# boqian333/E2ENet-Medical

Hardware: AMD Instinct MI355X
Metric: voxels/sec (train step fwd+bwd+update), 128^3 patch 32ch density=0.2 (higher is better)
Workload: dtype f32 (fp16x2 split products, f32 accumulate); 1 GPU; BraTS-shaped 4-modal 128^3 patches, shiftConvPP base 32, K=4, DSFF density 0.2, batch 2 per GPU, fwd+loss+bwd+clip+SGD+mask step, dense (parity) wgrad; parallelism=dp1

## Files before the change

e2enet_medical_amd/_lib.py:

```python
import ctypes as C
import os

_HERE = os.path.dirname(os.path.abspath(__file__))
LIB_PATH = os.environ.get("E2E_LIB_PATH") or os.path.join(_HERE, "csrc", "libe2e_hip.so")

KNOWN_ENV = frozenset({
    "E2E_CONV_MM", "E2E_MM_GRID", "E2E_MM_GEOM", "E2E_MM_PAIRQ", "E2E_CONV_DENSE", "E2E_CONV_SPARSE2", "E2E_CONV_PERSIST", "E2E_CONV_WGS",
    "E2E_CONV_KSPLIT", "E2E_WG_H2", "E2E_WG_BF3", "E2E_CT_BF3", "E2E_CT_H2",
    "E2E_CONV_DBG", "E2E_MM_STAMPS",
    "E2E_LIB_PATH", "E2E_STRICT_ENV", "E2E_DENSE_MIN_DENSITY", "E2E_MM_MIN_DENSITY", "E2E_WGRAD_STREAM", "E2E_LANES", "E2E_GRAPHS",
    "E2E_GRAPH_MAX_VOXELS", "E2E_PLAN_CACHE_GB", "E2E_SW_BLOCKING", "E2E_FORCE_DIST",
    "E2E_CPU_THREADS", "E2E_BENCH_DRY", "E2E_BENCH_DRY_FAIL_RANK", "E2E_BENCH_ALL_LAUNCHES",
})


def check_env(environ=None, strict=None):
    environ = os.environ if environ is None else environ
    unknown = sorted(k for k in environ if k.startswith("E2E_") and k not in KNOWN_ENV)
    if not unknown:
        return
    msg = ("unknown E2E_* environment variable(s) %s: not read by this build (known: %s)"
           % (", ".join(unknown), ", ".join(sorted(KNOWN_ENV))))
    if strict is None:
        strict = environ.get("E2E_STRICT_ENV") == "1"
    if strict:
        raise RuntimeError(msg)
    import warnings
    warnings.warn(msg + "; set E2E_STRICT_ENV=1 to refuse instead", RuntimeWarning, stacklevel=2)


class InChan(C.Structure):
    _fields_ = [("ptr", C.c_void_p), ("scale", C.c_void_p), ("shift", C.c_void_p),
                ("nstride", C.c_longlong), ("ab_nstride", C.c_int), ("dshift", C.c_int),
                ("slope", C.c_float), ("reserved", C.c_int)]


class OutChan(C.Structure):
    _fields_ = [("ptr", C.c_void_p), ("nstride", C.c_longlong), ("dshift", C.c_int), ("accumulate", C.c_int)]


class InSumChan(C.Structure):
    _fields_ = [("y", C.c_void_p), ("scale", C.c_void_p), ("shift", C.c_void_p), ("mean", C.c_void_p), ("rstd", C.c_void_p),
                ("part", C.c_void_p), ("nstride", C.c_longlong), ("part_nstride", C.c_longlong), ("ab_nstride", C.c_int),
                ("slope", C.c_float)]


class ParamEntry(C.Structure):
    _fields_ = [("param", C.c_void_p), ("grad", C.c_void_p), ("momentum", C.c_void_p), ("mask", C.c_void_p),
                ("numel", C.c_longlong)]


class SparsePackJob(C.Structure):
    _fields_ = [("w", C.c_void_p), ("wpk", C.c_void_p), ("qslot", C.c_void_p), ("pslot", C.c_void_p), ("quads", C.c_void_p),
                ("woff", C.c_void_p), ("groups", C.c_int), ("nchunks", C.c_int), ("wq_stride", C.c_int), ("wp_stride", C.c_int),
                ("reverse", C.c_int), ("kmax", C.c_int)]


class MmPackJob(C.Structure):
    _fields_ = [("w", C.c_void_p), ("quads", C.c_void_p), ("wpk", C.c_void_p), ("w_absmax", C.c_void_p), ("P", C.c_int), ("Q", C.c_int),
                ("wq_stride", C.c_int), ("wp_stride", C.c_int), ("reverse", C.c_int), ("owns_absmax", C.c_int)]


class RangeSrc(C.Structure):
    _fields_ = [("kind", C.c_int), ("C", C.c_int), ("N", C.c_longlong), ("gamma", C.c_void_p), ("beta", C.c_void_p), ("w", C.c_void_p),
                ("wCout", C.c_int), ("wks", C.c_int), ("word", C.c_void_p)]


class RangeJob(C.Structure):
    _fields_ = [("src", RangeSrc * 3), ("out", C.c_void_p)]


assert C.sizeof(MmPackJob) == 56 and C.sizeof(RangeSrc) == 56 and C.sizeof(RangeJob) == 176
assert C.sizeof(InChan) == 48 and C.sizeof(OutChan) == 24 and C.sizeof(ParamEntry) == 40 and C.sizeof(SparsePackJob) == 72 and C.sizeof(InSumChan) == 72

P, I, F, LL = C.c_void_p, C.c_int, C.c_float, C.c_longlong

SIGNATURES = {
    "e2e_last_error": (C.c_char_p, []),
    "e2e_abi_version": (I, []),
    "e2e_last_kernel": (C.c_char_p, []),
    "e2e_conv133_num_partials": (I, [I, I, I, I, I]),
    "e2e_conv133_fwd": (I, [P, I, P, P, P, P, P, I, I, I, I, I, I, I, I, P]),
    "e2e_conv133_fwd_ws_bytes": (LL, [I, I, I, I, I, I, I, I, I]),
    "e2e_conv133_fwd_splitk": (I, [P, I, P, P, P, P, P, I, I, I, I, I, I, I, I, P, LL, P]),
    "e2e_conv133_dgrad": (I, [P, P, P, P, I, I, I, I, I, I, I, I, I, P]),
    "e2e_conv133_dgrad_ws_bytes": (LL, [I, I, I, I, I, I, I, I, I]),
    "e2e_conv133_dgrad_splitk": (I, [P, P, P, P, I, I, I, I, I, I, I, I, I, P, LL, P]),
    "e2e_conv133_dense_ws_bytes": (LL, [I, I, I, I, I, I, I, I, I]),
    "e2e_conv133_sparse_eligible": (I, [I, I, I, I, I, I, I, I]),
    "e2e_conv133_sparse_wpk_floats": (LL, [I, I, I]),
    "e2e_conv133_sparse_plan": (I, [P, I, I, I, P, P, P, P, P, P]),
# ... 150 lines not shown
```

e2enet_medical_amd/csrc/conv133.hip:

```cpp
#include "e2e_common.h"
#include "e2e_split.h"
#include <cstdlib>
#include <cstdio>
#include <type_traits>

#ifdef E2E_CONV_DEBUG
#define CDBG(bit) ((p.dbg & (bit)) != 0)
__device__ unsigned long long g_conv_stamps[1024 * 8];
#define STAMP(var) const unsigned long long var = __builtin_readcyclecounter()
#define STAMP_ADD(i, a, b) st_acc[i] += (b) - (a)
#else
#define STAMP(var)
#define STAMP_ADD(i, a, b)
#define CDBG(bit) false
#endif

namespace {

using namespace e2e;

struct ConvParams {
  const e2e_in_chan_t* chans;
  const float* xin;
  const float* w;
// ... 984 lines not shown
  const bool vec = (DH == 1 && DW == 1) && (p.Wi % 4 == 0);
  switch (kind) {
    case 0:
      if (vec && opw8_knob() == 1 && p.P > 8) return launch_cfg<MODE, 1, 1, 1, 1, 16, 32, 8, 8, 8, 4, 8, 1, 3, 0>(p, st);
      if (vec && opw8_knob() == 2 && p.P > 8) return launch_cfg<MODE, 1, 1, 1, 1, 16, 32, 8, 8, 4, 4, 8, 1, 4, 0>(p, st);
      return vec ? launch_cfg<MODE, 1, 1, 1, 1, 16, 32, 8, 8, 4, 8, 8, 1, 4, 0>(p, st)
                 : launch_cfg<MODE, 1, 1, DH, DW, 16, 32, 8, 8, 4, 8, 8, 0, 4, 0>(p, st);
    case 1:
      return vec ? launch_cfg<MODE, 1, 1, 1, 1, 16, 16, 8, 8, 4, 8, 16, 1>(p, st)
                 : launch_cfg<MODE, 1, 1, DH, DW, 16, 16, 8, 8, 4, 8, 16, 0>(p, st);
    default:
      return vec ? launch_cfg<MODE, 1, 1, 1, 1, 8, 8, 8, 8, 4, 8, 16, 1>(p, st)
                 : launch_cfg<MODE, 1, 1, DH, DW, 8, 8, 8, 8, 4, 8, 16, 0>(p, st);
  }
}

enum TileKind { T32 = 0, T16 = 1, T8 = 2, T16x32S = 3, T8S = 4 };
inline TileKind pick_tile(int Ho, int Wo, int sh, int sw) {
  const bool strided = (sh != 1 || sw != 1);
  const int m = Ho < Wo ? Ho : Wo;
  if (strided) return m > 8 ? T16x32S : T8S;
  if (m > 16) return T32;
  if (m > 8) return T16;
  return T8;
}
inline void tile_dims(TileKind k, int& th, int& tw) {
  switch (k) {
    case T32: th = 16; tw = 32; break;
    case T16: th = 16; tw = 16; break;
    case T8: th = 8; tw = 8; break;
    case T16x32S: th = 16; tw = 32; break;
    default: th = 8; tw = 8; break;
  }
}



int launch_sub(const ConvParams& p, int kind, hipStream_t st) {
  const bool vec = (p.Ws % 4) == 0;
  if (kind == 0)
    return vec ? launch_cfg<2, 1, 1, 1, 1, 16, 32, 8, 8, 4, 8, 8, 1, 4, 0>(p, st)
               : launch_cfg<2, 1, 1, 1, 1, 16, 32, 8, 8, 4, 8, 8, 0, 4, 0>(p, st);
  return vec ? launch_cfg<2, 1, 1, 1, 1, 16, 16, 8, 8, 4, 8, 16, 1>(p, st)
             : launch_cfg<2, 1, 1, 1, 1, 16, 16, 8, 8, 4, 8, 16, 0>(p, st);
}

}

extern "C" int e2e_conv133_num_partials(int Do, int Ho, int Wo, int sh, int sw) {
  int th, tw;
  tile_dims(pick_tile(Ho, Wo, sh, sw), th, tw);
  return Do * e2e::cdiv(Ho, th) * e2e::cdiv(Wo, tw);
}

static int plan_fwd_ksplit(int B, int Cin, int Cout, int Di, int Hi, int Wi, int sd, int sh, int sw) {
  static const int knob = getenv("E2E_CONV_KSPLIT") ? atoi(getenv("E2E_CONV_KSPLIT")) : -1;
  const int Do = (Di - 1) / sd + 1, Ho = (Hi - 1) / sh + 1, Wo = (Wi - 1) / sw + 1;
  const TileKind k = pick_tile(Ho, Wo, sh, sw);
  if (k == T32 || k == T16x32S) return 1;
  int th, tw;
  tile_dims(k, th, tw);
  const int chunks = e2e::cdiv(Cin, 16);
  const long long base = (long long)B * Do * e2e::cdiv(Ho, th) * e2e::cdiv(Wo, tw) * e2e::cdiv(Cout, 32);
  if (knob == 0 || knob == 1) return 1;
  long long ks = knob > 1 ? knob : 1024 / (base > 0 ? base : 1);
  if (ks > 8) ks = 8;
  if (ks > chunks / 2) ks = chunks / 2;
  return ks < 2 ? 1 : (int)ks;
}

extern "C" long long e2e_conv133_fwd_ws_bytes(int B, int Cin, int Cout, int Di, int Hi, int Wi, int sd, int sh, int sw) {
  const int ks = plan_fwd_ksplit(B, Cin, Cout, Di, Hi, Wi, sd, sh, sw);
  if (ks <= 1) return 0;
  const long long Do = (Di - 1) / sd + 1, Ho = (Hi - 1) / sh + 1, Wo = (Wi - 1) / sw + 1;
  return (long long)ks * B * Cout * Do * Ho * Wo * 4;
}

static int conv133_fwd_impl(const e2e_in_chan_t* chans, int Cin, const float* w, const float* bias, const unsigned* live, float* y,
                            double* part, int B, int Cout, int Di, int Hi, int Wi, int sd, int sh, int sw, float* ws,
                            long long ws_bytes, void* stream) {
  E2E_REQUIRE(chans && w && y, "conv133_fwd: null pointer");
  E2E_REQUIRE(B > 0 && Cin > 0 && Cout > 0 && Di > 0 && Hi > 0 && Wi > 0, "conv133_fwd: bad dims");
  E2E_REQUIRE((sd == 1 || sd == 2) && (sh == 1 || sh == 2) && (sw == 1 || sw == 2), "conv133_fwd: stride must be 1 or 2");
  ConvParams p{};
  p.chans = chans; p.xin = nullptr; p.w = w; p.bias = bias; p.live = live; p.y = y; p.part = part; p.outs = nullptr;
  p.P = Cin; p.Q = Cout; p.wq_stride = Cin * 9; p.wp_stride = 9; p.live_words = e2e::cdiv(Cin, 32);
  p.B = B; p.Di = Di; p.Hi = Hi; p.Wi = Wi; p.sd = sd;
  p.Do = (Di - 1) / sd + 1; p.Ho = (Hi - 1) / sh + 1; p.Wo = (Wi - 1) / sw + 1;
  p.Ds = Di; p.Hs = Hi; p.Ws = Wi;
  p.ksplit = 1; p.kpart = nullptr;
  if (ws != nullptr) {
    const long long need = e2e_conv133_fwd_ws_bytes(B, Cin, Cout, Di, Hi, Wi, sd, sh, sw);
    if (need > 0) {
      E2E_REQUIRE(ws_bytes >= need, "conv133_fwd: workspace too small (%lld < %lld bytes)", ws_bytes, need);
      p.ksplit = plan_fwd_ksplit(B, Cin, Cout, Di, Hi, Wi, sd, sh, sw);
      p.kpart = ws;
    }
  }
  hipStream_t st = (hipStream_t)stream;
  const TileKind k = pick_tile(p.Ho, p.Wo, sh, sw);
  if (sh == 1 && sw == 1) return launch_s1<0, 1, 1>(p, k == T32 ? 0 : (k == T16 ? 1 : 2), st);
  if (sh == 2 && sw == 2) {
    if (k == T16x32S && (Wi % 4) == 0) return launch_cfg<0, 2, 2, 1, 1, 16, 32, 4, 16, 4, 8, 8, 1>(p, st);
    if (k == T16x32S) return launch_cfg<0, 2, 2, 1, 1, 16, 32, 4, 16, 4, 8, 8, 0>(p, st);
    return launch_cfg<0, 2, 2, 1, 1, 8, 8, 8, 8, 4, 8, 16, 0>(p, st);
  }
  if (sh == 1 && sw == 2) {
    if (k == T16x32S) return launch_cfg<0, 1, 2, 1, 1, 16, 32, 4, 16, 4, 8, 8, 0>(p, st);
    return launch_cfg<0, 1, 2, 1, 1, 8, 8, 8, 8, 4, 8, 16, 0>(p, st);
  }
  if (k == T16x32S) return launch_cfg<0, 2, 1, 1, 1, 16, 32, 4, 16, 4, 8, 8, 0>(p, st);
  return launch_cfg<0, 2, 1, 1, 1, 8, 8, 8, 8, 4, 8, 16, 0>(p, st);
}

extern "C" int e2e_conv133_fwd(const e2e_in_chan_t* chans, int Cin, const float* w, const float* bias,
                               const unsigned* live, float* y, double* part, int B, int Cout, int Di, int Hi, int Wi,
                               int sd, int sh, int sw, void* stream) {
  return conv133_fwd_impl(chans, Cin, w, bias, live, y, part, B, Cout, Di, Hi, Wi, sd, sh, sw, nullptr, 0, stream);
}

extern "C" int e2e_conv133_fwd_splitk(const e2e_in_chan_t* chans, int Cin, const float* w, const float* bias,
                                      const unsigned* live, float* y, double* part, int B, int Cout, int Di, int Hi, int Wi,
                                      int sd, int sh, int sw, float* ws, long long ws_bytes, void* stream) {
  return conv133_fwd_impl(chans, Cin, w, bias, live, y, part, B, Cout, Di, Hi, Wi, sd, sh, sw, ws, ws_bytes, stream);
}

static int plan_dgrad_ksplit(int B, int Cin, int Cout, int Di, int Hi, int Wi, int sd, int sh, int sw) {
  static const int knob = getenv("E2E_CONV_KSPLIT") ? atoi(getenv("E2E_CONV_KSPLIT")) : -1;
  if (knob == 0 || knob == 1) return 1;
  const bool tiled = (sh == 1 && sw == 1) || (sh == 2 && sw == 2);
  if (!tiled) return 1;
  const TileKind k = pick_tile(Hi, Wi, 1, 1);
  if (k == T32) return 1;
  int th, tw;
  tile_dims(k, th, tw);
  const int chunks = e2e::cdiv(Cout, 16);
  const long long base = (long long)B * Di * e2e::cdiv(Hi, th) * e2e::cdiv(Wi, tw) * e2e::cdiv(Cin, 32);
  long long ks = knob > 1 ? knob : 1024 / (base > 0 ? base : 1);
  if (ks > 8) ks = 8;
  if (ks > chunks / 2) ks = chunks / 2;
  return ks < 2 ? 1 : (int)ks;
}

extern "C" long long e2e_conv133_dgrad_ws_bytes(int B, int Cin, int Cout, int Di, int Hi, int Wi, int sd, int sh, int sw) {
  const int ks = plan_dgrad_ksplit(B, Cin, Cout, Di, Hi, Wi, sd, sh, sw);
  return ks <= 1 ? 0 : (long long)ks * B * Cin * Di * Hi * Wi * 4;
}

static int conv133_dgrad_impl(const float* dy, const float* w, const unsigned* live_t, const e2e_out_chan_t* outs,
                              int B, int Cin, int Cout, int Di, int Hi, int Wi, int sd, int sh, int sw, float* ws,
                              long long ws_bytes, void* stream) {
  E2E_REQUIRE(dy && w && outs, "conv133_dgrad: null pointer");
  E2E_REQUIRE(B > 0 && Cin > 0 && Cout > 0 && Di > 0 && Hi > 0 && Wi > 0, "conv133_dgrad: bad dims");
  E2E_REQUIRE((sd == 1 || sd == 2) && (sh == 1 || sh == 2) && (sw == 1 || sw == 2), "conv133_dgrad: stride must be 1 or 2");
  hipStream_t st = (hipStream_t)stream;
  const int Do = (Di - 1) / sd + 1, Ho = (Hi - 1) / sh + 1, Wo = (Wi - 1) / sw + 1;
  const bool tiled = (sh == 1 && sw == 1) || (sh == 2 && sw == 2);
  if (!tiled) {
    const long long per = (long long)Di * Hi * Wi;
    dim3 grid((unsigned)e2e::cdivll(per, 256), Cin, B);
    e2e::note_kernel("conv133_dgrad_strided_gather");
    hipLaunchKernelGGL(conv133_dgrad_strided_kernel, grid, dim3(256), 0, st, dy, w, outs, B, Cin, Cout, Di, Hi, Wi, Do,
                       Ho, Wo, sd, sh, sw);
    return e2e::check_launch("conv133_dgrad_strided_kernel");
  }
  ConvParams p{};
  p.chans = nullptr; p.xin = dy; p.w = w; p.bias = nullptr; p.live = live_t; p.y = nullptr; p.part = nullptr; p.outs = outs;
  p.P = Cout; p.Q = Cin; p.wq_stride = 9; p.wp_stride = Cin * 9; p.live_words = e2e::cdiv(Cout, 32);
  p.B = B; p.Di = Di; p.Hi = Hi; p.Wi = Wi; p.sd = sd; p.Do = Di; p.Ho = Hi; p.Wo = Wi;
  p.Ds = Do; p.Hs = Ho; p.Ws = Wo;
  p.ksplit = 1; p.kpart = nullptr;
  if (ws != nullptr) {
    const long long need = e2e_conv133_dgrad_ws_bytes(B, Cin, Cout, Di, Hi, Wi, sd, sh, sw);
    if (need > 0) {
      E2E_REQUIRE(ws_bytes >= need, "conv133_dgrad: workspace too small (%lld < %lld bytes)", ws_bytes, need);
      p.ksplit = plan_dgrad_ksplit(B, Cin, Cout, Di, Hi, Wi, sd, sh, sw);
      p.kpart = ws;
    }
  }
  const TileKind k = pick_tile(Hi, Wi, 1, 1);
  const int kind = k == T32 ? 0 : (k == T16 ? 1 : 2);
  if (sh == 1) return launch_s1<1, 1, 1>(p, kind, st);
  if (kind <= 1 && (Hi % 2) == 0 && (Wi % 2) == 0) {
    p.wq_stride = 9; p.wp_stride = Cin * 9;
    return launch_sub(p, kind, st);
  }
  return launch_s1<1, 2, 2>(p, kind, st);
}

extern "C" int e2e_conv133_dgrad(const float* dy, const float* w, const unsigned* live_t, const e2e_out_chan_t* outs,
                                 int B, int Cin, int Cout, int Di, int Hi, int Wi, int sd, int sh, int sw,
                                 void* stream) {
  return conv133_dgrad_impl(dy, w, live_t, outs, B, Cin, Cout, Di, Hi, Wi, sd, sh, sw, nullptr, 0, stream);
}

extern "C" int e2e_conv133_dgrad_splitk(const float* dy, const float* w, const unsigned* live_t, const e2e_out_chan_t* outs,
                                        int B, int Cin, int Cout, int Di, int Hi, int Wi, int sd, int sh, int sw, float* ws,
                                        long long ws_bytes, void* stream) {
  return conv133_dgrad_impl(dy, w, live_t, outs, B, Cin, Cout, Di, Hi, Wi, sd, sh, sw, ws, ws_bytes, stream);
}
```

e2enet_medical_amd/csrc/e2e_common.h:

```cpp
#pragma once
#include <hip/hip_runtime.h>
#include <cstdio>
#include <cstdarg>
#include "e2e_hip.h"

typedef const float __attribute__((address_space(1)))* gfloat_p;

namespace e2e {

void set_error(const char* fmt, ...);
void note_kernel(const char* fmt, ...);

void mm_clock_read(unsigned long long out[2], bool reset);
void wgrad_clock_read(unsigned long long out[2], bool reset);

inline int check_launch(const char* what) {
  hipError_t e = hipGetLastError();
  if (e != hipSuccess) {
    set_error("%s: %s", what, hipGetErrorString(e));
    return E2E_ERR_LAUNCH;
  }
  return E2E_OK;
}

// ... 7 lines not shown

__host__ __device__ inline int cdiv(int a, int b) { return (a + b - 1) / b; }
__host__ __device__ inline long long cdivll(long long a, long long b) { return (a + b - 1) / b; }

__device__ __forceinline__ float in_act(float v, float a, float b, float slope) {
  float u = fmaf(v, a, b);
  return u > 0.f ? u : u * slope;
}

__device__ __forceinline__ float wave_sum_dpp(float v) {
  v += __builtin_bit_cast(float, __builtin_amdgcn_update_dpp(0, __builtin_bit_cast(int, v), 0xB1, 0xF, 0xF, true));
  v += __builtin_bit_cast(float, __builtin_amdgcn_update_dpp(0, __builtin_bit_cast(int, v), 0x4E, 0xF, 0xF, true));
  v += __builtin_bit_cast(float, __builtin_amdgcn_update_dpp(0, __builtin_bit_cast(int, v), 0x141, 0xF, 0xF, true));
  v += __builtin_bit_cast(float, __builtin_amdgcn_update_dpp(0, __builtin_bit_cast(int, v), 0x140, 0xF, 0xF, true));
  v += __shfl_xor(v, 16, 64);
  v += __shfl_xor(v, 32, 64);
  return v;
}

__device__ __forceinline__ double dpp_move_d(double v, const int ctrl_sel) {
  const long long b = __builtin_bit_cast(long long, v);
  int lo = (int)b, hi = (int)(b >> 32);
  switch (ctrl_sel) {
    case 0: lo = __builtin_amdgcn_update_dpp(0, lo, 0xB1, 0xF, 0xF, true); hi = __builtin_amdgcn_update_dpp(0, hi, 0xB1, 0xF, 0xF, true); break;
    case 1: lo = __builtin_amdgcn_update_dpp(0, lo, 0x4E, 0xF, 0xF, true); hi = __builtin_amdgcn_update_dpp(0, hi, 0x4E, 0xF, 0xF, true); break;
    case 2: lo = __builtin_amdgcn_update_dpp(0, lo, 0x141, 0xF, 0xF, true); hi = __builtin_amdgcn_update_dpp(0, hi, 0x141, 0xF, 0xF, true); break;
    default: lo = __builtin_amdgcn_update_dpp(0, lo, 0x140, 0xF, 0xF, true); hi = __builtin_amdgcn_update_dpp(0, hi, 0x140, 0xF, 0xF, true); break;
  }
  return __builtin_bit_cast(double, ((long long)hi << 32) | (unsigned)lo);
}
__device__ __forceinline__ double wave_sum_dpp_d(double v) {
  v += dpp_move_d(v, 0);
  v += dpp_move_d(v, 1);
  v += dpp_move_d(v, 2);
  v += dpp_move_d(v, 3);
  v += __shfl_xor(v, 16, 64);
  v += __shfl_xor(v, 32, 64);
  return v;
}

__device__ __forceinline__ float wave_sum(float v) {
#pragma unroll
  for (int off = 32; off > 0; off >>= 1) v += __shfl_xor(v, off, 64);
  return v;
}
__device__ __forceinline__ double wave_sum_d(double v) {
#pragma unroll
  for (int off = 32; off > 0; off >>= 1) v += __shfl_xor(v, off, 64);
  return v;
}

__device__ __forceinline__ int xcd_remap(int id, int padded_total) {
  int per = padded_total >> 3;
  return (id & 7) * per + (id >> 3);
}

__global__ inline void zero_words_kernel(unsigned* p, long long n) {
  for (long long i = (long long)blockIdx.x * blockDim.x + threadIdx.x; i < n; i += (long long)gridDim.x * blockDim.x) p[i] = 0u;
}
inline void zero_async(void* p, size_t bytes, hipStream_t st) {
  const long long n = (long long)(bytes / 4);
  long long blocks = (n + 255) / 256;
  if (blocks > 2048) blocks = 2048;
  if (blocks < 1) blocks = 1;
  hipLaunchKernelGGL(zero_words_kernel, dim3((unsigned)blocks), dim3(256), 0, st, (unsigned*)p, n);
}

struct WgBf3Params {
  const e2e_in_chan_t* chans;
  const float* dy;
  float* slab;
  int B, Cin, Cout, Di, Hi, Wi, Do, sd;
  int tiles_x, tiles_y, tiles_per_n, tiles_per_chunk;
  int segs;
  int cblocks;
  int geom;
  int h2;
  const unsigned* dy_absmax;
  const unsigned* x_absmax;
};
int launch_wgrad_bf3(const WgBf3Params& p, int nchunks, int pairs, hipStream_t st);
int reduce_slabs(const float* slab, float* dw, long long numel, int nslabs, hipStream_t st);

inline int split_tiles(long long total, int pairs, int target_wgs, int min_tiles, int* tiles_per_chunk) {
  long long want = target_wgs / (pairs > 0 ? pairs : 1);
  if (want < 1) want = 1;
  long long tpc = cdivll(total, want);
  if (tpc < min_tiles) tpc = min_tiles;
  if (tpc > total) tpc = total;
  *tiles_per_chunk = (int)tpc;
  return (int)cdivll(total, tpc);
}
inline int split_tiles_per_item(int tiles_per_n, int B, int pairs, int target_wgs, int min_tiles, int* tiles_per_chunk, int* segs) {
  long long want = target_wgs / (pairs > 0 ? pairs : 1);
  if (want < B) want = B;
  int tpc = cdiv(tiles_per_n, (int)(want / B));
  if (tpc < min_tiles) tpc = min_tiles;
  if (tpc > tiles_per_n) tpc = tiles_per_n;
  *tiles_per_chunk = tpc;
  *segs = cdiv(tiles_per_n, tpc);
  return *segs * B;
}

}
```

e2enet_medical_amd/engine.py:

```python
import contextlib
import ctypes as C
import math
import os
from typing import Dict, List, Optional, Sequence, Tuple

import torch

import numpy as np

from ._lib import lib, InChan, OutChan, ParamEntry, SparsePackJob, InSumChan, MmPackJob, RangeSrc, RangeJob

LRELU_SLOPE = 0.01
IN_EPS = 1e-5
DENSE_MIN_DENSITY = float(os.environ.get("E2E_DENSE_MIN_DENSITY", "0.5"))
WGRAD_STREAM = os.environ.get("E2E_WGRAD_STREAM", "1") != "0"
WGRAD_STREAM_MAX_ELEMS = 40000000
WGRAD_LATE = True
LANES = os.environ.get("E2E_LANES", "1") != "0"
LANE_DIVS = None


def _lane_divs(voxels):
    if LANE_DIVS is not None:
        return LANE_DIVS
# ... 655 lines not shown
        self._region_words_dev = {}
        self._mm_tables = {}
        self._mm_packed = {}
        self._range_table = None
        self._range_key = None
        self.weights_epoch = 0

    def _build_unetpp(self, cfg):
        P = cfg.num_pool
        nodes = {}
        cur = self.input
        for st in range(P + 1):
            stride = (1, 1, 1) if st == 0 else cfg.pool_kernels[st - 1]
            for bi, prefix in enumerate(cfg.encoder_prefixes(st)):
                op = self._add_conv(prefix, [cur], cfg.feats[st], stride if bi == 0 else (1, 1, 1))
                cur = op.out
            nodes[(st, 0)] = cur
            if st == 0:
                continue
            z = P - st
            for m, lvl in cfg.nest_nodes(z):
                j = st - lvl
                up = UpOp(self, "up%d.%d.weight" % (z, m), nodes[(lvl + 1, j - 1)], cfg.feats[lvl], cfg.pool_kernels[lvl])
                self.ops.append(up)
                self.up_ops[up.w_name] = up
                srcs = [nodes[(lvl, j - 1)], up.out]
                if lvl > 0:
                    pool = PoolOp(self, "down%d.%d" % (z, m), nodes[(lvl - 1, j - 1)], cfg.pool_kernels[lvl - 1])
                    self.ops.append(pool)
                    srcs.append(pool.out)
                t = None
                for prefix in cfg.loc_prefixes(z, m):
                    op = self._add_conv(prefix, srcs if t is None else [t], cfg.feats[lvl], (1, 1, 1))
                    t = op.out
                nodes[(lvl, j)] = t
        self.nodes = nodes
        for h in range(4):
            head = HeadOp(self, "seg_outputs.%d.weight" % h, nodes[(h, P - h)], cfg.num_classes)
            self.heads.append(head)
            self.ops.append(head)

    def _build_unet(self, cfg):
        P = cfg.num_pool
        skips, cur = [], self.input
        for st in range(P + 1):
            stride = (1, 1, 1) if st == 0 else cfg.pool_kernels[st - 1]
            for bi, prefix in enumerate(cfg.encoder_prefixes(st)):
                op = self._add_conv(prefix, [cur], cfg.feats[st], stride if bi == 0 else (1, 1, 1))
                cur = op.out
            if st < P:
                skips.append(cur)
        self.nodes = {(st, 0): a for st, a in enumerate(skips)}
        by_u = []
        for u in range(P):
            lvl = P - 1 - u
            up = UpOp(self, "tu.%d.weight" % u, cur, cfg.feats[lvl], cfg.pool_kernels[lvl])
            self.ops.append(up)
            self.up_ops[up.w_name] = up
            t = None
            for prefix in cfg.unet_loc_prefixes(u):
                op = self._add_conv(prefix, [up.out, skips[lvl]] if t is None else [t], cfg.feats[lvl], (1, 1, 1))
                t = op.out
            cur = t
            self.nodes[(lvl, 1)] = t
            head = HeadOp(self, "seg_outputs.%d.weight" % u, t, cfg.num_classes)
            self.ops.append(head)
            by_u.append(head)
        self.heads = [by_u[-1]] + by_u[:-1][::-1]

    def _add_conv(self, prefix, sources, cout, stride):
        op = ConvOp(self, prefix, sources, cout, stride)
        self.ops.append(op)
        self.conv_ops[op.w_name] = op
        return op

    def set_kernel_masks(self, kmasks: Dict[str, torch.Tensor]):
        L = lib()
        self.maps_generation += 1
        self._graphs.clear()
        self._graph_seen.clear()
        self._sparse_jobs = None
        for name, op in list(self.conv_ops.items()) + list(self.up_ops.items()):
            km = kmasks.get(name)
            if isinstance(op, ConvOp):
                op.build_sparse_plans(km)
            if km is None:
                op.live = op.live_t = None
                op.density = 1.0
                continue
            r, cc = km.shape
            op.density = float(km.float().mean().item())
            km = km.to(device=self.device, dtype=torch.uint8).contiguous()
            if isinstance(op, ConvOp):
                rows = torch.empty(((r + 3) // 4) * ((cc + 7) // 8), dtype=torch.int32, device=self.device)
                cols = torch.empty(((cc + 3) // 4) * ((r + 7) // 8), dtype=torch.int32, device=self.device)
                L.dsff_expand_quads(km.data_ptr(), rows.data_ptr(), cols.data_ptr(), r, cc, _stream())
                op.live, op.live_t = rows, cols
            else:
                rows = torch.empty(r * ((cc + 31) // 32), dtype=torch.int32, device=self.device)
                cols = torch.empty(cc * ((r + 31) // 32), dtype=torch.int32, device=self.device)
                L.dsff_expand(km.data_ptr(), None, rows.data_ptr(), cols.data_ptr(), r, cc, 1, _stream())
                op.live, op.live_t = cols, rows

    def kernel_masks_from_weights(self, names=None):
        L = lib()
        out = {}
        for name, op in list(self.conv_ops.items()) + list(self.up_ops.items()):
            if names is not None and name not in names:
                continue
            w = self.params[name]
            r, cc = w.shape[0], w.shape[1]
            ks = w[0, 0].numel()
            km = torch.empty((r, cc), dtype=torch.uint8, device=self.device)
            L.dsff_kmask_from_weights(w.data_ptr(), km.data_ptr(), r, cc, ks, _stream())
            out[name] = km
        return out

    def forward(self, x: torch.Tensor, deep_supervision: bool = True):
        assert x.is_cuda and x.dtype == torch.float32, "engine input must be a float32 GPU tensor"
        assert tuple(x.shape) == self.input.shape, "engine built for %s, got %s" % (self.input.shape, tuple(x.shape))
        if self.pre_forward_hook is not None:
            self.pre_forward_hook()
        self.input.data.copy_(x)
        self.generation += 1
        for h in self.heads:
            h.active = bool(deep_supervision) or h is self.heads[0]
        self._run(("fwd", bool(deep_supervision)), self._forward_ops)
        outs = [h.out.data for h in self.heads]
        return outs if deep_supervision else outs[0]

    def _pack_sparse(self):
        def matrix_only(op):
            return (op.use_mm("f") and op.use_mm("b")) or op.use_dense()
        key = tuple(matrix_only(op) for op in self.conv_ops.values())
        if self._sparse_jobs is None or self._sparse_jobs[0] != key:
            jobs = [j for op in self.conv_ops.values() if not matrix_only(op) for j in op.sparse_jobs()]
            self._sparse_jobs = (key, pack_sparse_weights(jobs, self.device) or ())
        if self._sparse_jobs[1]:
            table, n, mx = self._sparse_jobs[1]
            lib().conv133_sparse_pack(table.data_ptr(), n, mx, _stream())

    def weights_changed(self):
        self.weights_epoch += 1

    def _weights_key(self):
        ptrs = tuple(p.data_ptr() for p in self.params.values())
        return ptrs, (PARAM_EPOCH, self.weights_epoch, self.maps_generation, tuple(p._version for p in self.params.values()))

    def _refresh_weight_caches(self, directions):
        L = lib()
        ptrs, state = self._weights_key()
        always = self._graph_ok() or torch.cuda.is_current_stream_capturing()
        if self.input_absmax is not None and "f" in directions:
            L.absmax_word(self.input.data.data_ptr(), self.input.data.numel(), self.input_absmax.data_ptr(), _stream())
        if always or self._range_key != (ptrs, state):
            if self._range_table is None or self._range_table[2] != ptrs:
                jobs = []
                for op in self.conv_ops.values():
                    jb = op.range_job()
                    op.range_known = jb is not None
                    if jb is not None:
                        jobs.append(jb)
                for up in self.up_ops.values():
                    jbs = up.range_jobs()
                    up.ranges_known = jbs is not None
                    if jbs is not None:
# ... 370 lines not shown
```

Before: 129.0 million voxels/s.

## Add MFMA kernels for dense stride-2 conv133 forward and dgrad

Adds dedicated bf16-split (three-term) MFMA kernels for the 1x3x3 conv with 2x2 spatial stride, in both forward (with fused instance-norm stats) and data-gradient directions. They are used when the layer has no live mask, replacing the generic tiled or strided-gather paths. The engine also treats all-ones kernel masks as dense so these layers can take the new path. The cost is a large amount of new kernel code whose output must match the old paths, including boundary handling and accumulate/zero-fill modes.

```diff
diff --git a/e2enet_medical_amd/_lib.py b/e2enet_medical_amd/_lib.py
--- a/e2enet_medical_amd/_lib.py
+++ b/e2enet_medical_amd/_lib.py
@@ -6,7 +6,7 @@
 
 KNOWN_ENV = frozenset({
     "E2E_CONV_MM", "E2E_MM_GRID", "E2E_MM_GEOM", "E2E_MM_PAIRQ", "E2E_CONV_DENSE", "E2E_CONV_SPARSE2", "E2E_CONV_PERSIST", "E2E_CONV_WGS",
-    "E2E_CONV_KSPLIT", "E2E_WG_H2", "E2E_WG_BF3", "E2E_CT_BF3", "E2E_CT_H2",
+    "E2E_CONV_KSPLIT", "E2E_CONV_S2MM", "E2E_WG_H2", "E2E_WG_BF3", "E2E_CT_BF3", "E2E_CT_H2",
     "E2E_CONV_DBG", "E2E_MM_STAMPS",
     "E2E_LIB_PATH", "E2E_STRICT_ENV", "E2E_DENSE_MIN_DENSITY", "E2E_MM_MIN_DENSITY", "E2E_WGRAD_STREAM", "E2E_LANES", "E2E_GRAPHS",
     "E2E_GRAPH_MAX_VOXELS", "E2E_PLAN_CACHE_GB", "E2E_SW_BLOCKING", "E2E_FORCE_DIST",
diff --git a/e2enet_medical_amd/csrc/conv133.hip b/e2enet_medical_amd/csrc/conv133.hip
--- a/e2enet_medical_amd/csrc/conv133.hip
+++ b/e2enet_medical_amd/csrc/conv133.hip
@@ -1090,6 +1090,8 @@
   E2E_REQUIRE(chans && w && y, "conv133_fwd: null pointer");
   E2E_REQUIRE(B > 0 && Cin > 0 && Cout > 0 && Di > 0 && Hi > 0 && Wi > 0, "conv133_fwd: bad dims");
   E2E_REQUIRE((sd == 1 || sd == 2) && (sh == 1 || sh == 2) && (sw == 1 || sw == 2), "conv133_fwd: stride must be 1 or 2");
+  if (e2e::conv133_s2mm_serves(live, Cin, Hi, Wi, sh, sw))
+    return e2e::launch_conv133_s2mm_fwd(chans, Cin, w, bias, y, part, B, Cout, Di, Hi, Wi, sd, (hipStream_t)stream);
   ConvParams p{};
   p.chans = chans; p.xin = nullptr; p.w = w; p.bias = bias; p.live = live; p.y = y; p.part = part; p.outs = nullptr;
   p.P = Cin; p.Q = Cout; p.wq_stride = Cin * 9; p.wp_stride = 9; p.live_words = e2e::cdiv(Cin, 32);
@@ -1163,6 +1165,8 @@
   E2E_REQUIRE((sd == 1 || sd == 2) && (sh == 1 || sh == 2) && (sw == 1 || sw == 2), "conv133_dgrad: stride must be 1 or 2");
   hipStream_t st = (hipStream_t)stream;
   const int Do = (Di - 1) / sd + 1, Ho = (Hi - 1) / sh + 1, Wo = (Wi - 1) / sw + 1;
+  if (e2e::conv133_s2mm_serves(live_t, Cin, Hi, Wi, sh, sw))
+    return e2e::launch_conv133_s2mm_dgrad(dy, w, outs, B, Cin, Cout, Di, Hi, Wi, sd, st);
   const bool tiled = (sh == 1 && sw == 1) || (sh == 2 && sw == 2);
   if (!tiled) {
     const long long per = (long long)Di * Hi * Wi;
diff --git a/e2enet_medical_amd/csrc/conv133_s2mm.hip b/e2enet_medical_amd/csrc/conv133_s2mm.hip
--- /dev/null
+++ b/e2enet_medical_amd/csrc/conv133_s2mm.hip
@@ -0,0 +1,525 @@
+#include "e2e_common.h"
+#include "e2e_split.h"
+#include <cstdlib>
+
+namespace {
+
+using namespace e2e;
+
+constexpr int NT = 512;
+constexpr int BR = 4, XR = 2 * BR + 1, XC = 65;
+constexpr int PXB = 32;
+constexpr int SPL = XR * XC * PXB;
+constexpr int XBYTES = 3 * SPL;
+constexpr int XG = 17;
+constexpr int NITEM = XR * XG;
+constexpr int QW = 64;
+constexpr int WROW = QW * 32;
+constexpr int WBYTES = 27 * WROW;
+constexpr int CTAB_MAX = 256, CTAB_ENT = 24;
+constexpr int SPITCH = 36;
+static_assert(XBYTES + WBYTES + 16 * QW * 2 * 4 + CTAB_MAX * CTAB_ENT <= 163840, "one workgroup per CU");
+static_assert(8 * 32 * SPITCH * 4 <= XBYTES, "the epilogue staging (8 waves x 32 channels x 32 pixels fp32) fits the input image");
+static_assert(QW * 8 == NT, "weight staging: one (out channel, channel pair) per thread");
+
+struct S2Params {
+  const e2e_in_chan_t* chans;
+  const float* w;
+  const float* bias;
+  float* y;
+  double* part;
+  int P, Q, B, Di, Hi, Wi, Do, Ho, Wo, sd;
+  int nchunks, qgroups, tiles_x, tiles_y, tiles_per_n, total, padded_total;
+};
+
+constexpr f32x16_t ZERO16 = {0.f, 0.f, 0.f, 0.f, 0.f, 0.f, 0.f, 0.f, 0.f, 0.f, 0.f, 0.f, 0.f, 0.f, 0.f, 0.f};
+
+__device__ __forceinline__ int slot_off(int slot, int half) { return slot * PXB + ((half ^ ((slot >> 3) & 1)) << 4); }
+
+__global__ __launch_bounds__(NT) void conv133_s2mm_fwd_kernel(S2Params p) {
+  __shared__ __attribute__((aligned(16))) unsigned char lds[XBYTES];
+  __shared__ __attribute__((aligned(16))) unsigned char wlds[WBYTES];
+  __shared__ float red[16][QW][2];
+  __shared__ __attribute__((aligned(8))) unsigned char ctab[CTAB_MAX * CTAB_ENT];
+
+  const int tid = threadIdx.x, lane = tid & 63;
+  const int wave = __builtin_amdgcn_readfirstlane(tid >> 6);
+  int item = e2e::xcd_remap(blockIdx.x, p.padded_total);
+  if (item >= p.total) return;
+  const int qg = item % p.qgroups;
+  item /= p.qgroups;
+  const int n = item / p.tiles_per_n, tile_in_n = item - n * p.tiles_per_n;
+  const int tx = tile_in_n % p.tiles_x, ty = (tile_in_n / p.tiles_x) % p.tiles_y, d = tile_in_n / (p.tiles_x * p.tiles_y);
+  const int h0 = ty * 16, w0 = tx * 32, q0 = qg * QW;
+  const long long in_plane = (long long)p.Hi * p.Wi, out_plane = (long long)p.Ho * p.Wo;
+  const int nb = (p.Ho - h0 + BR - 1) / BR < 4 ? (p.Ho - h0 + BR - 1) / BR : 4;
+
+  const int shalf = wave >> 2;
+  const int sitem = tid & 255;
+  const bool s_act = sitem < NITEM;
+  const int s_row = (s_act ? sitem : 0) / XG, s_g = (s_act ? sitem : 0) - s_row * XG;
+  const int s_rslot = (s_row & 1) ? (s_row - 1) / 2 : BR + s_row / 2;
+  int s_off = -1;
+  auto set_geometry = [&](int band) {
+    const int hi = 2 * (h0 + BR * band) - 1 + s_row, wi = 2 * w0 - 4 + 4 * s_g;
+    const bool ok = s_act && (unsigned)hi < (unsigned)p.Hi && wi >= 0 && wi < p.Wi;
+    s_off = ok ? hi * p.Wi + wi : -1;
+  };
+  f32x4_t xv[8];
+  unsigned pvalid = 0;
+  auto prefetch_x = [&](int c) {
+    gfloat_p base[8];
+    pvalid = 0;
+#pragma unroll
+    for (int j = 0; j < 8; ++j) {
+      const unsigned char* e = ctab + (c * 16 + shalf * 8 + j) * CTAB_ENT;
+      base[j] = (gfloat_p)(*reinterpret_cast<const unsigned long long*>(e));
+      pvalid |= (*reinterpret_cast<const unsigned*>(e + 20) & 1u) << j;
+    }
+    const int off = s_off >= 0 ? s_off : 0;
+#pragma unroll
+    for (int j = 0; j < 8; ++j) xv[j] = *(gf4_p)(unsigned long long)(base[j] + off);
+  };
+  auto commit_x = [&](int c) {
+    if (!s_act) return;
+    const bool inside = s_off >= 0;
+    float pa[8], pb[8], psl[8];
+#pragma unroll
+    for (int j = 0; j < 8; ++j) {
+      const unsigned char* e = ctab + (c * 16 + shalf * 8 + j) * CTAB_ENT;
+      const float2 ab = *reinterpret_cast<const float2*>(e + 8);
+      pa[j] = ab.x; pb[j] = ab.y;
+      psl[j] = *reinterpret_cast<const float*>(e + 16);
+    }
+#pragma unroll
+    for (int k = 0; k < 4; ++k) {
+      const int rel = 4 * s_g + k - 3;
+      if (rel < 0) continue;
+      const int cslot = (rel & 1) ? (rel - 1) / 2 : 32 + rel / 2;
+      unsigned hh[8], mm[8], ll[8];
+#pragma unroll
+      for (int j = 0; j < 8; ++j) {
+        float v = e2e::in_act(xv[j][k], pa[j], pb[j], psl[j]);
+        v = (((pvalid >> j) & 1u) && inside) ? v : 0.f;
+        split_bf3(v, hh[j], mm[j], ll[j]);
+      }
+      unsigned char* dst = lds + slot_off(s_rslot * XC + cslot, shalf);
+      *reinterpret_cast<u32x4_t*>(dst) = u32x4_t{pack_hi16(hh[0], hh[1]), pack_hi16(hh[2], hh[3]), pack_hi16(hh[4], hh[5]), pack_hi16(hh[6], hh[7])};
+      *reinterpret_cast<u32x4_t*>(dst + SPL) = u32x4_t{pack_hi16(mm[0], mm[1]), pack_hi16(mm[2], mm[3]), pack_hi16(mm[4], mm[5]), pack_hi16(mm[6], mm[7])};
+      *reinterpret_cast<u32x4_t*>(dst + 2 * SPL) = u32x4_t{pack_hi16(ll[0], ll[1]), pack_hi16(ll[2], ll[3]), pack_hi16(ll[4], ll[5]), pack_hi16(ll[6], ll[7])};
+    }
+  };
+
+  float wv[9][2];
+  const int w_ql = tid >> 3, w_pp = tid & 7;
+  auto prefetch_w = [&](int c) {
+    const int q = q0 + w_ql, ch = c * 16 + 2 * w_pp;
+    const bool ok0 = q < p.Q && ch < p.P, ok1 = q < p.Q && ch + 1 < p.P;
+    const float* src = p.w + ((long long)(ok0 ? q : 0) * p.P + (ok0 ? ch : 0)) * 9;
+#pragma unroll
+    for (int t = 0; t < 9; ++t) {
+      wv[t][0] = ok0 ? src[t] : 0.f;
+      wv[t][1] = ok1 ? src[9 + t] : 0.f;
+    }
+  };
+  auto commit_w = [&]() {
+    unsigned char* dst = wlds + slot_off(w_ql, w_pp >> 2) + (w_pp & 3) * 4;
+#pragma unroll
+    for (int t = 0; t < 9; ++t) {
+      unsigned h0w, m0w, l0w, h1w, m1w, l1w;
+      split_bf3(wv[t][0], h0w, m0w, l0w);
+      split_bf3(wv[t][1], h1w, m1w, l1w);
+      *reinterpret_cast<unsigned*>(dst + (t * 3) * WROW) = pack_hi16(h0w, h1w);
+      *reinterpret_cast<unsigned*>(dst + (t * 3 + 1) * WROW) = pack_hi16(m0w, m1w);
+      *reinterpret_cast<unsigned*>(dst + (t * 3 + 2) * WROW) = pack_hi16(l0w, l1w);
+    }
+  };
+
+  const int fq = lane & 31, fh8 = lane >> 5;
+  const int row = wave & 3, qblk = wave >> 2;
+  const unsigned char* const wfbase = wlds + slot_off(qblk * 32 + fq, fh8);
+  int aoff[9];
+#pragma unroll
+  for (int t = 0; t < 9; ++t) {
+    const int kh = t / 3, kw = t - kh * 3;
+    const int rslot = kh == 1 ? row : BR + row + (kh == 2 ? 1 : 0);
+    const int cslot = kw == 1 ? 0 : 32 + (kw == 2 ? 1 : 0);
+    aoff[t] = slot_off(rslot * XC + cslot + fq, fh8);
+  }
+  const int q_lane = q0 + qblk * 32 + fq;
+  const float bq = (p.bias != nullptr && q_lane < p.Q) ? p.bias[q_lane] : 0.f;
+
+  set_geometry(0);
+  prefetch_w(0);
+  for (int ch = tid; ch < p.nchunks * 16; ch += NT) {
+    const e2e_in_chan_t cd = p.chans[ch < p.P ? ch : 0];
+    const int din = d * p.sd - cd.dshift;
+    const bool valid = ch < p.P && (unsigned)din < (unsigned)p.Di;
+    float a = 1.f, b = 0.f, sl = 1.f;
+    if (cd.scale != nullptr) {
+      a = cd.scale[(long long)n * cd.ab_nstride];
+      b = cd.shift[(long long)n * cd.ab_nstride];
+      sl = cd.slope;
+    }
+    unsigned char* e = ctab + ch * CTAB_ENT;
+    *reinterpret_cast<unsigned long long*>(e) = (unsigned long long)(cd.ptr + (long long)n * cd.nstride + (long long)(valid ? din : 0) * in_plane);
+    *reinterpret_cast<float2*>(e + 8) = float2{a, b};
+    *reinterpret_cast<float*>(e + 16) = sl;
+    *reinterpret_cast<unsigned*>(e + 20) = valid ? 1u : 0u;
+  }
+  __syncthreads();
+  prefetch_x(0);
+
+  f32x16_t acc[4];
+#pragma unroll
+  for (int b = 0; b < 4; ++b)
+#pragma unroll
+    for (int i = 0; i < 16; ++i) acc[b][i] = 0.f;
+
+  for (int c = 0; c < p.nchunks; ++c) {
+#pragma unroll
+    for (int b = 0; b < 4; ++b) {
+      if (b >= nb) continue;
+      if (b == 0) commit_w();
+      commit_x(c);
+      __syncthreads();
+      if (b + 1 < nb) { set_geometry(b + 1); prefetch_x(c); }
+      else if (c + 1 < p.nchunks) { set_geometry(0); prefetch_w(c + 1); prefetch_x(c + 1); }
+      if (h0 + BR * b + row < p.Ho) {
+        f32x16_t a = acc[b];
+#pragma unroll
+        for (int t = 0; t < 9; ++t) {
+          bf16x8_t af[3], wb[3];
+#pragma unroll
+          for (int s = 0; s < 3; ++s) {
+            af[s] = *reinterpret_cast<const bf16x8_t*>(lds + aoff[t] + s * SPL);
+            wb[s] = *reinterpret_cast<const bf16x8_t*>(wfbase + (t * 3 + s) * WROW);
+          }
+          f32x16_t tp = ZERO16;
+          tp = __builtin_amdgcn_mfma_f32_32x32x16_bf16(af[2], wb[0], tp, 0, 0, 0);
+          tp = __builtin_amdgcn_mfma_f32_32x32x16_bf16(af[1], wb[1], tp, 0, 0, 0);
+          tp = __builtin_amdgcn_mfma_f32_32x32x16_bf16(af[0], wb[2], tp, 0, 0, 0);
+          tp = __builtin_amdgcn_mfma_f32_32x32x16_bf16(af[1], wb[0], tp, 0, 0, 0);
+          tp = __builtin_amdgcn_mfma_f32_32x32x16_bf16(af[0], wb[1], tp, 0, 0, 0);
+          tp = __builtin_amdgcn_mfma_f32_32x32x16_bf16(af[0], wb[0], tp, 0, 0, 0);
+          a += tp;
+        }
+        acc[b] = a;
+      }
+      __syncthreads();
+    }
+  }
+
+  float* const stg = reinterpret_cast<float*>(lds) + wave * 32 * SPITCH;
+  const int vc = p.Wo - w0 < 32 ? p.Wo - w0 : 32;
+#pragma unroll
+  for (int b = 0; b < 4; ++b) {
+    const int oh = h0 + BR * b + row;
+    if (oh >= p.Ho) continue;
+    float psum = 0.f;
+#pragma unroll
+    for (int i = 0; i < 16; ++i) {
+      acc[b][i] += bq;
+      const bool ok = (i & 3) + 8 * (i >> 2) + 4 * fh8 < vc;
+      psum += ok ? acc[b][i] : 0.f;
+    }
+    if (p.part != nullptr) {
+      const float mean = (psum + __shfl_xor(psum, 32, 64)) / (float)vc;
+      float m2 = 0.f;
+#pragma unroll
+      for (int i = 0; i < 16; ++i) {
+        const bool ok = (i & 3) + 8 * (i >> 2) + 4 * fh8 < vc;
+        const float dl = ok ? acc[b][i] - mean : 0.f;
+        m2 = fmaf(dl, dl, m2);
+      }
+      m2 += __shfl_xor(m2, 32, 64);
+      if (fh8 == 0) { red[b * 4 + row][qblk * 32 + fq][0] = mean; red[b * 4 + row][qblk * 32 + fq][1] = m2; }
+    }
+#pragma unroll
+    for (int g = 0; g < 4; ++g)
+      *reinterpret_cast<f32x4_t*>(stg + fq * SPITCH + 4 * fh8 + 8 * g) = f32x4_t{acc[b][4 * g], acc[b][4 * g + 1], acc[b][4 * g + 2], acc[b][4 * g + 3]};
+#pragma unroll
+    for (int k = 0; k < 4; ++k) {
+      const int ql = 8 * k + (lane >> 3), px4 = (lane & 7) * 4;
+      const int q = q0 + qblk * 32 + ql;
+      const f32x4_t v = *reinterpret_cast<const f32x4_t*>(stg + ql * SPITCH + px4);
+      if (q >= p.Q || px4 >= vc) continue;
+      *reinterpret_cast<f32x4_t*>(p.y + (((long long)n * p.Q + q) * p.Do + d) * out_plane + (long long)oh * p.Wo + w0 + px4) = v;
+    }
+  }
+  __syncthreads();
+  if (p.part != nullptr && tid < QW && q0 + tid < p.Q) {
+    double cn = 0.0, cm = 0.0, c2 = 0.0;
+    for (int k = 0; k < 16; ++k) {
+      if (h0 + k >= p.Ho) break;
+      const double bn = (double)vc, bm = (double)red[k][tid][0], b2 = (double)red[k][tid][1];
+      const double tot = cn + bn, dl = bm - cm;
+      cm += dl * (bn / tot);
+      c2 += b2 + dl * dl * (cn * bn / tot);
+      cn = tot;
+    }
+    double* pp = p.part + (((long long)n * p.Q + q0 + tid) * p.tiles_per_n + tile_in_n) * 3;
+    pp[0] = cn; pp[1] = cm; pp[2] = c2;
+  }
+}
+
+constexpr int DR = 8, DXR = DR + 1, DXC = 33;
+constexpr int DSPL = DXR * DXC * PXB;
+constexpr int DXBYTES = 3 * DSPL;
+constexpr int DXG = 9;
+constexpr int DNITEM = DXR * DXG;
+constexpr int DWROW = 32 * 32;
+constexpr int DWBYTES = 27 * DWROW;
+static_assert(8 * 32 * SPITCH * 4 <= DXBYTES + DWBYTES, "the epilogue staging fits the image and the weights");
+
+struct S2DParams {
+  const float* dy;
+  const float* w;
+  const e2e_out_chan_t* outs;
+  int P, Q, B, Di, Hi, Wi, Ds, Hs, Ws, sd;
+  int nchunks, qblocks, tiles_x, tiles_y, tiles_per_n, total, padded_total;
+};
+
+__global__ __launch_bounds__(NT) void conv133_s2mm_dgrad_kernel(S2DParams p) {
+  __shared__ __attribute__((aligned(16))) unsigned char smem[DXBYTES + DWBYTES];
+  unsigned char* const lds = smem;
+  unsigned char* const wlds = smem + DXBYTES;
+
+  const int tid = threadIdx.x, lane = tid & 63;
+  const int wave = __builtin_amdgcn_readfirstlane(tid >> 6);
+  int item = e2e::xcd_remap(blockIdx.x, p.padded_total);
+  if (item >= p.total) return;
+  const int qb = item % p.qblocks;
+  item /= p.qblocks;
+  const int n = item / p.tiles_per_n, tile_in_n = item - n * p.tiles_per_n;
+  const int tx = tile_in_n % p.tiles_x, ty = (tile_in_n / p.tiles_x) % p.tiles_y, d = tile_in_n / (p.tiles_x * p.tiles_y);
+  const int h0 = ty * DR, w0 = tx * 32, q0 = qb * 32;
+  const long long src_plane = (long long)p.Hs * p.Ws, out_plane = (long long)p.Hi * p.Wi;
+  const int nchunks = (d % p.sd) == 0 ? p.nchunks : 0;
+  const int dsrc = d / p.sd;
+
+  const int squart = wave >> 1;
+  const int sitem = tid & 127;
+  const bool s_act = sitem < DNITEM;
+  const int s_row = (s_act ? sitem : 0) / DXG, s_g = (s_act ? sitem : 0) - s_row * DXG;
+  int s_off = -1;
+  {
+    const int hy = h0 + s_row, wy = w0 + 4 * s_g;
+    if (s_act && hy < p.Hs && wy < p.Ws) s_off = hy * p.Ws + wy;
+  }
+  f32x4_t xv[4];
+  unsigned pvalid = 0;
+  auto prefetch_x = [&](int c) {
+    pvalid = 0;
+    const int off = s_off >= 0 ? s_off : 0;
+#pragma unroll
+    for (int j = 0; j < 4; ++j) {
+      const int ch = c * 16 + squart * 4 + j;
+      const bool v = ch < p.P;
+      pvalid |= (v ? 1u : 0u) << j;
+      const float* base = p.dy + (((long long)n * p.P + (v ? ch : 0)) * p.Ds + dsrc) * src_plane;
+      xv[j] = *(gf4_p)(unsigned long long)(base + off);
+    }
+  };
+  auto commit_x = [&]() {
+    if (!s_act) return;
+    const bool inside = s_off >= 0;
+#pragma unroll
+    for (int k = 0; k < 4; ++k) {
+      const int col = 4 * s_g + k;
+      if (col >= DXC) continue;
+      unsigned hh[4], mm[4], ll[4];
+#pragma unroll
+      for (int j = 0; j < 4; ++j) {
+        const float v = (((pvalid >> j) & 1u) && inside) ? xv[j][k] : 0.f;
+        split_bf3(v, hh[j], mm[j], ll[j]);
+      }
+      unsigned char* dst = lds + slot_off(s_row * DXC + col, squart >> 1) + (squart & 1) * 8;
+      *reinterpret_cast<u32x2_t*>(dst) = u32x2_t{pack_hi16(hh[0], hh[1]), pack_hi16(hh[2], hh[3])};
+      *reinterpret_cast<u32x2_t*>(dst + DSPL) = u32x2_t{pack_hi16(mm[0], mm[1]), pack_hi16(mm[2], mm[3])};
+      *reinterpret_cast<u32x2_t*>(dst + 2 * DSPL) = u32x2_t{pack_hi16(ll[0], ll[1]), pack_hi16(ll[2], ll[3])};
+    }
+  };
+
+  float wv[5][2];
+  const int w_cl = tid >> 4, w_pp = (tid >> 1) & 7, w_t0 = (tid & 1) * 5;
+  auto prefetch_w = [&](int c) {
+    const int q = q0 + w_cl, ch = c * 16 + 2 * w_pp;
+    const bool ok0 = q < p.Q && ch < p.P, ok1 = q < p.Q && ch + 1 < p.P;
+    const float* src = p.w + ((long long)(ok0 ? ch : 0) * p.Q + (ok0 ? q : 0)) * 9 + w_t0;
+    const long long ostride = (long long)p.Q * 9;
+#pragma unroll
+    for (int t = 0; t < 5; ++t) {
+      const bool tk = w_t0 + t < 9;
+      wv[t][0] = (ok0 && tk) ? src[t] : 0.f;
+      wv[t][1] = (ok1 && tk) ? src[ostride + t] : 0.f;
+    }
+  };
+  auto commit_w = [&]() {
+    unsigned char* dst = wlds + w_t0 * 3 * DWROW + slot_off(w_cl, w_pp >> 2) + (w_pp & 3) * 4;
+#pragma unroll
+    for (int t = 0; t < 5; ++t) {
+      if (w_t0 + t >= 9) continue;
+      unsigned h0w, m0w, l0w, h1w, m1w, l1w;
+      split_bf3(wv[t][0], h0w, m0w, l0w);
+      split_bf3(wv[t][1], h1w, m1w, l1w);
+      *reinterpret_cast<unsigned*>(dst + (t * 3) * DWROW) = pack_hi16(h0w, h1w);
+      *reinterpret_cast<unsigned*>(dst + (t * 3 + 1) * DWROW) = pack_hi16(m0w, m1w);
+      *reinterpret_cast<unsigned*>(dst + (t * 3 + 2) * DWROW) = pack_hi16(l0w, l1w);
+    }
+  };
+
+  const int fq = lane & 31, fh8 = lane >> 5;
+  const unsigned char* const wfbase = wlds + slot_off(fq, fh8);
+  int aoff[4];
+#pragma unroll
+  for (int t = 0; t < 4; ++t) aoff[t] = slot_off((wave + (t >> 1)) * DXC + fq + (t & 1), fh8);
+
+  float* dptr[4];
+  int dmode[4];
+#pragma unroll
+  for (int k = 0; k < 4; ++k) {
+    const int q = q0 + 8 * k + (lane >> 3);
+    dptr[k] = nullptr; dmode[k] = 0;
+    if (q >= p.Q) continue;
+    const e2e_out_chan_t oc = p.outs[q];
+    if (oc.ptr == nullptr) continue;
+    int dd = d - oc.dshift;
+    bool zero_fill = false;
+    if (dd < 0) {
+      const int lo = p.Di - oc.dshift > 0 ? p.Di - oc.dshift : 0;
+      dd = lo + d;
+      zero_fill = true;
+    } else if (dd >= p.Di) {
+      const int lo = p.Di + oc.dshift > 0 ? p.Di + oc.dshift : 0;
+      dd = d - lo;
+      zero_fill = true;
+    }
+    if (oc.accumulate && (zero_fill || nchunks == 0)) continue;
+    dptr[k] = oc.ptr + (long long)n * oc.nstride + (long long)dd * out_plane;
+    dmode[k] = zero_fill ? 2 : (oc.accumulate ? 1 : 0);
+  }
+
+  f32x16_t acc[4];
+#pragma unroll
+  for (int b = 0; b < 4; ++b)
+#pragma unroll
+    for (int i = 0; i < 16; ++i) acc[b][i] = 0.f;
+
+  if (nchunks > 0) { prefetch_w(0); prefetch_x(0); }
+  for (int c = 0; c < nchunks; ++c) {
+    commit_w();
+    commit_x();
+    __syncthreads();
+    if (c + 1 < nchunks) { prefetch_w(c + 1); prefetch_x(c + 1); }
+    if (h0 + wave < p.Hs) {
+#pragma unroll
+      for (int t = 0; t < 9; ++t) {
+        const int kh = t / 3, kw = t - kh * 3;
+        const int cls = (kh == 1 ? 0 : 2) + (kw == 1 ? 0 : 1);
+        const int ao = aoff[(kh == 0 ? 2 : 0) + (kw == 0 ? 1 : 0)];
+        bf16x8_t af[3], wb[3];
+#pragma unroll
+        for (int s = 0; s < 3; ++s) {
+          af[s] = *reinterpret_cast<const bf16x8_t*>(lds + ao + s * DSPL);
+          wb[s] = *reinterpret_cast<const bf16x8_t*>(wfbase + (t * 3 + s) * DWROW);
+        }
+        f32x16_t a = acc[cls];
+        f32x16_t tp = ZERO16;
+        tp = __builtin_amdgcn_mfma_f32_32x32x16_bf16(af[2], wb[0], tp, 0, 0, 0);
+        tp = __builtin_amdgcn_mfma_f32_32x32x16_bf16(af[1], wb[1], tp, 0, 0, 0);
+        tp = __builtin_amdgcn_mfma_f32_32x32x16_bf16(af[0], wb[2], tp, 0, 0, 0);
+        tp = __builtin_amdgcn_mfma_f32_32x32x16_bf16(af[1], wb[0], tp, 0, 0, 0);
+        tp = __builtin_amdgcn_mfma_f32_32x32x16_bf16(af[0], wb[1], tp, 0, 0, 0);
+        tp = __builtin_amdgcn_mfma_f32_32x32x16_bf16(af[0], wb[0], tp, 0, 0, 0);
+        a += tp;
+        acc[cls] = a;
+      }
+    }
+    __syncthreads();
+  }
+
+  if (h0 + wave >= p.Hs) return;
+  float* const stg = reinterpret_cast<float*>(smem) + wave * 32 * SPITCH;
+#pragma unroll
+  for (int pi = 0; pi < 2; ++pi) {
+    const int oh = 2 * (h0 + wave) + pi;
+#pragma unroll
+    for (int hc = 0; hc < 2; ++hc) {
+      if (2 * w0 + 32 * hc >= p.Wi) continue;
+#pragma unroll
+      for (int i = 0; i < 8; ++i) {
+        const int px = (i & 3) + 8 * (i >> 2) + 4 * fh8;
+        *reinterpret_cast<f32x2_t*>(stg + fq * SPITCH + 2 * px) = f32x2_t{acc[pi * 2][8 * hc + i], acc[pi * 2 + 1][8 * hc + i]};
+      }
+      const long long po = (long long)oh * p.Wi + 2 * w0 + 32 * hc + (lane & 7) * 4;
+      f32x4_t v[4], old[4];
+#pragma unroll
+      for (int k = 0; k < 4; ++k) {
+        v[k] = *reinterpret_cast<const f32x4_t*>(stg + (8 * k + (lane >> 3)) * SPITCH + (lane & 7) * 4);
+        old[k] = f32x4_t{0.f, 0.f, 0.f, 0.f};
+        if (dptr[k] != nullptr && dmode[k] == 1) old[k] = *reinterpret_cast<const f32x4_t*>(dptr[k] + po);
+      }
+#pragma unroll
+      for (int k = 0; k < 4; ++k) {
+        if (dptr[k] == nullptr) continue;
+        f32x4_t o = dmode[k] == 2 ? f32x4_t{0.f, 0.f, 0.f, 0.f} : v[k];
+        o += old[k];
+        *reinterpret_cast<f32x4_t*>(dptr[k] + po) = o;
+      }
+    }
+  }
+}
+
+inline bool s2mm_knob() {
+  static const int mm = getenv("E2E_CONV_MM") ? atoi(getenv("E2E_CONV_MM")) : 1;
+  static const int s2 = getenv("E2E_CONV_S2MM") ? atoi(getenv("E2E_CONV_S2MM")) : 1;
+  return mm != 0 && s2 != 0;
+}
+
+}
+
+namespace e2e {
+
+bool conv133_s2mm_serves(const void* live, int Cin, int Hi, int Wi, int sh, int sw) {
+  if (!s2mm_knob() || live != nullptr || sh != 2 || sw != 2) return false;
+  if ((Hi & 1) || (Wi & 1)) return false;
+  const int Ho = Hi / 2, Wo = Wi / 2;
+  return Wo % 16 == 0 && (Ho < Wo ? Ho : Wo) > 8 && Cin <= CTAB_MAX;
+}
+
+int launch_conv133_s2mm_fwd(const e2e_in_chan_t* chans, int Cin, const float* w, const float* bias, float* y, double* part, int B, int Cout,
+                            int Di, int Hi, int Wi, int sd, hipStream_t st) {
+  S2Params p{};
+  p.chans = chans; p.w = w; p.bias = bias; p.y = y; p.part = part;
+  p.P = Cin; p.Q = Cout; p.B = B; p.Di = Di; p.Hi = Hi; p.Wi = Wi; p.sd = sd;
+  p.Do = (Di - 1) / sd + 1; p.Ho = Hi / 2; p.Wo = Wi / 2;
+  p.nchunks = cdiv(Cin, 16);
+  p.qgroups = cdiv(Cout, QW);
+  p.tiles_x = cdiv(p.Wo, 32); p.tiles_y = cdiv(p.Ho, 16);
+  p.tiles_per_n = p.Do * p.tiles_y * p.tiles_x;
+  p.total = B * p.tiles_per_n * p.qgroups;
+  p.padded_total = (p.total + 7) & ~7;
+  note_kernel("conv133_s2mm<mode=0,s=2x2,tile=16x32> wgs=%d chunks=%d", p.padded_total, p.nchunks);
+  hipLaunchKernelGGL(conv133_s2mm_fwd_kernel, dim3(p.padded_total), dim3(NT), 0, st, p);
+  return check_launch("conv133_s2mm_fwd_kernel");
+}
+
+int launch_conv133_s2mm_dgrad(const float* dy, const float* w, const e2e_out_chan_t* outs, int B, int Cin, int Cout, int Di, int Hi, int Wi,
+                              int sd, hipStream_t st) {
+  S2DParams p{};
+  p.dy = dy; p.w = w; p.outs = outs;
+  p.P = Cout; p.Q = Cin; p.B = B; p.Di = Di; p.Hi = Hi; p.Wi = Wi; p.sd = sd;
+  p.Ds = (Di - 1) / sd + 1; p.Hs = Hi / 2; p.Ws = Wi / 2;
+  p.nchunks = cdiv(Cout, 16);
+  p.qblocks = cdiv(Cin, 32);
+  p.tiles_x = cdiv(p.Ws, 32); p.tiles_y = cdiv(p.Hs, DR);
+  p.tiles_per_n = Di * p.tiles_y * p.tiles_x;
+  p.total = B * p.tiles_per_n * p.qblocks;
+  p.padded_total = (p.total + 7) & ~7;
+  note_kernel("conv133_s2mm<mode=2,s=2x2,tile=16x64> wgs=%d chunks=%d", p.padded_total, p.nchunks);
+  hipLaunchKernelGGL(conv133_s2mm_dgrad_kernel, dim3(p.padded_total), dim3(NT), 0, st, p);
+  return check_launch("conv133_s2mm_dgrad_kernel");
+}
+
+}
diff --git a/e2enet_medical_amd/csrc/e2e_common.h b/e2enet_medical_amd/csrc/e2e_common.h
--- a/e2enet_medical_amd/csrc/e2e_common.h
+++ b/e2enet_medical_amd/csrc/e2e_common.h
@@ -113,6 +113,12 @@
 int launch_wgrad_bf3(const WgBf3Params& p, int nchunks, int pairs, hipStream_t st);
 int reduce_slabs(const float* slab, float* dw, long long numel, int nslabs, hipStream_t st);
 
+bool conv133_s2mm_serves(const void* live, int Cin, int Hi, int Wi, int sh, int sw);
+int launch_conv133_s2mm_fwd(const e2e_in_chan_t* chans, int Cin, const float* w, const float* bias, float* y, double* part, int B, int Cout,
+                            int Di, int Hi, int Wi, int sd, hipStream_t st);
+int launch_conv133_s2mm_dgrad(const float* dy, const float* w, const e2e_out_chan_t* outs, int B, int Cin, int Cout, int Di, int Hi, int Wi,
+                              int sd, hipStream_t st);
+
 inline int split_tiles(long long total, int pairs, int target_wgs, int min_tiles, int* tiles_per_chunk) {
   long long want = target_wgs / (pairs > 0 ? pairs : 1);
   if (want < 1) want = 1;
diff --git a/e2enet_medical_amd/engine.py b/e2enet_medical_amd/engine.py
--- a/e2enet_medical_amd/engine.py
+++ b/e2enet_medical_amd/engine.py
@@ -761,6 +761,8 @@
         self._sparse_jobs = None
         for name, op in list(self.conv_ops.items()) + list(self.up_ops.items()):
             km = kmasks.get(name)
+            if km is not None and bool(km.all()):
+                km = None
             if isinstance(op, ConvOp):
                 op.build_sparse_plans(km)
             if km is None:
```

Result: faster. 131.1 million voxels/s (median of 6 runs) (+1.6%).
